# aik2mlj/polyffusion

Hardware: AMD Instinct MI355X
Metric: denoising steps/sec (8-bar prmat2c, batch 16) (higher is better)
Workload: dtype bf16x3; 1 GPU; sdf_chd8bar cond generation, batch 16 per GPU, 1000-step DDPM sampler loop body (BASELINE.json configs[1]); weights: deterministic synthetic, 41.08M params; global_batch=16, parallelism=batch-shard x1

## Files before the change

### polyffusion_amd/csrc/conv_common.h

```cpp
#pragma once
#include <type_traits>

#include "pf_internal.h"

namespace pf {

typedef x3_t x3x8 __attribute__((ext_vector_type(8)));
typedef unsigned int u32x4 __attribute__((ext_vector_type(4)));

template <int OFF>
__device__ __forceinline__ x3x8 lds_read128(unsigned addr) {
  u32x4 v;
  constexpr int HI = OFF & ~0xFFFF, LO = OFF & 0xFFFF;
  if constexpr (HI != 0) addr += HI;
  asm volatile("ds_read_b128 %0, %1 offset:%2" : "=v"(v) : "v"(addr), "n"(LO));
  return __builtin_bit_cast(x3x8, v);
}
__device__ __forceinline__ __amdgpu_buffer_rsrc_t dma_resource(const void* base) {
  return __builtin_amdgcn_make_buffer_rsrc(const_cast<void*>(base), 0, 0x7fffffff, 0x00020000);
}
__device__ __forceinline__ void dma16(__amdgpu_buffer_rsrc_t rs, int voff, int soff, void* lds_wave_base) {
  __builtin_amdgcn_raw_ptr_buffer_load_lds(rs, (__attribute__((address_space(3))) void*)lds_wave_base, 16, voff, soff, 0, 0);
}

template <int N>
__device__ __forceinline__ void lgkm_wait() { asm volatile("s_waitcnt lgkmcnt(%0)" ::"n"(N)); }
template <int I, int N, class F>
__device__ __forceinline__ void static_for(F&& f) {
  if constexpr (I < N) { f(std::integral_constant<int, I>{}); static_for<I + 1, N>(f); }
}


struct FastDiv { unsigned mul, shr; };
static inline FastDiv make_fastdiv(int d) {
  if (d <= 1) return FastDiv{0u, 0u};
  unsigned l = 31u - (unsigned)__builtin_clz((unsigned)d);
  if (d & (d - 1)) ++l;
  const unsigned p = 31u + l;
  return FastDiv{(unsigned)(((1ull << p) + (unsigned)d - 1u) / (unsigned)d), p - 32u};
}
__device__ __forceinline__ int fdiv(int x, FastDiv f) { return f.mul ? (int)(__umulhi((unsigned)x, f.mul) >> f.shr) : x; }

struct ConvP {
  const float* x0; const float* x1; int c0, c1;
  int B, Hin, Win, Hout, Wout;
  const void* w; int N, Npad;
  const float* sc; const float* sh; const float* mean; const float* rstd;
  const float* bias; const float* sbias; int ld_sbias; const float* res; int ld_res;
  const long long* sb_rows; int sb_nrows;
  int geglu;
  float* out; int ld_out;
  float* stats;
  int tiles_x, tiles_y, nt;
  FastDiv d_tx, d_ty, d_nt, d_ks;
  int fold, fold_py, fold_px;
  const float* sx0; const float* sx1; int sc0, sc1;
  const void* sw; const float* bias2;
  void* out_planes;
  void* qkv;
  int pp;
  int ksplit; float* partial;
  const float* gn_s0; const float* gn_s1; int gn_t0, gn_t1;
  const float* gn_gamma; const float* gn_beta; float gn_eps; int gn_groups;
  int x1_bmod;
  unsigned* amax;
  int pad_br;
};

__device__ __forceinline__ void conv_shared_x1(ConvP& p, int b) {
  if (p.x1_bmod > 0) {
    const size_t d = (size_t)(b - b % p.x1_bmod);
    if (p.x1) p.x1 -= d * ((size_t)p.Hin * p.Win * p.c1);
    if (p.sx1) p.sx1 -= d * ((size_t)p.Hout * p.Wout * p.sc1);
    if (p.gn_s1) p.gn_s1 -= d * ((size_t)p.gn_t1 * p.c1 * 2);
  }
}

static inline void conv_fill_divs(ConvP& p) {
  p.d_tx = make_fastdiv(p.tiles_x); p.d_ty = make_fastdiv(p.tiles_y); p.d_nt = make_fastdiv(p.nt); p.d_ks = make_fastdiv(p.ksplit);
}

template <int NTHREADS>
__device__ __forceinline__ void gn_fused_prologue(const ConvP& p, int b, int tid_wg, int hw, double* scratch) {
  const int cin = p.c0 + p.c1, gs = cin / p.gn_groups;
  for (int c = tid_wg; c < cin; c += NTHREADS) {
    const float* s; int T, C, cl;
    if (c < p.c0) { s = p.gn_s0; T = p.gn_t0; C = p.c0; cl = c; } else { s = p.gn_s1; T = p.gn_t1; C = p.c1; cl = c - p.c0; }
    double a = 0.0, q = 0.0;
    for (int t0 = 0; t0 < T; t0 += 8) {
      float2 vv[8];
#pragma unroll
      for (int j = 0; j < 8; ++j)
        vv[j] = *reinterpret_cast<const float2*>(s + (((size_t)b * T + min(t0 + j, T - 1)) * C + cl) * 2);
#pragma unroll
      for (int j = 0; j < 8; ++j)
        if (t0 + j < T) { a += vv[j].x; q += vv[j].y; }
    }
    scratch[2 * c] = a; scratch[2 * c + 1] = q;
  }
  __syncthreads();
  float* scw = const_cast<float*>(p.sc) + (size_t)b * cin;
  float* shw = const_cast<float*>(p.sh) + (size_t)b * cin;
  for (int c = tid_wg; c < cin; c += NTHREADS) {
    const int g0 = (c / gs) * gs;
    double a = 0.0, q = 0.0;
    for (int j = 0; j < gs; ++j) { a += scratch[2 * (g0 + j)]; q += scratch[2 * (g0 + j) + 1]; }
    const double cnt = (double)gs * hw;
    const double mean = a / cnt;
    double var = q / cnt - mean * mean;
    if (var < 0.0) var = 0.0;
    const double rstd = 1.0 / sqrt(var + (double)p.gn_eps);
    const double ga = p.gn_gamma[c];
    scw[c] = (float)(rstd * ga);
    shw[c] = (float)((double)p.gn_beta[c] - mean * rstd * ga);
  }
  __threadfence_block();
  __syncthreads();
}

__device__ __forceinline__ void amax_acc(unsigned& m, float v) { m = max(m, __float_as_uint(v) & 0x7fffffffu); }
__device__ __forceinline__ void amax_acc4(unsigned& m, f32x4 v) { amax_acc(m, v[0]); amax_acc(m, v[1]); amax_acc(m, v[2]); amax_acc(m, v[3]); }
__device__ __forceinline__ void amax_flush(unsigned* slot, unsigned m) {
  if (!slot) return;
#pragma unroll
  for (int o = 32; o >= 1; o >>= 1) m = max(m, (unsigned)__shfl_xor((int)m, o));
  if ((threadIdx.x & 63) == 0 && m) atomicMax(slot, m);
}

__device__ __forceinline__ float silu_f(float v) { return v * __builtin_amdgcn_rcpf(1.0f + __expf(-v)); }
__device__ __forceinline__ float erf_as_f(float x) {
  const float ax = fabsf(x);
  const float t = __builtin_amdgcn_rcpf(fmaf(0.3275911f, ax, 1.0f));
  float pq = fmaf(1.061405429f, t, -1.453152027f);
  pq = fmaf(pq, t, 1.421413741f);
  pq = fmaf(pq, t, -0.284496736f);
  pq = fmaf(pq, t, 0.254829592f);
  const float y = 1.0f - pq * t * __expf(-ax * ax);
  return copysignf(y, x);
}
__device__ __forceinline__ float gelu_erf_f(float g) { return 0.5f * g * (1.0f + erf_as_f(g * 0.70710678118654752440f)); }

__device__ __forceinline__ void store_out(const ConvP& p, size_t idx, float v) { p.out[idx] = v; }
__device__ __forceinline__ const float* sbias_row(const ConvP& p, int b) {
  if (!p.sbias) return nullptr;
  long long r = b;
  if (p.sb_rows) { r = p.sb_rows[b]; r = r < 0 ? 0 : (r >= p.sb_nrows ? p.sb_nrows - 1 : r); }
  return p.sbias + (size_t)r * p.ld_sbias;
}
__device__ __forceinline__ size_t out_pixel(const ConvP& p, int b, int oy, int ox) {
  if (p.fold) return ((size_t)b * (2 * p.Hout) + 2 * oy + p.fold_py) * (size_t)(2 * p.Wout) + 2 * ox + p.fold_px;
  return ((size_t)b * p.Hout + oy) * p.Wout + ox;
}

__device__ __forceinline__ void quad_transpose_s1(f32x4& a, int lane) {
  const bool p1 = lane & 1;
  float s0 = p1 ? a[0] : a[1], s1 = p1 ? a[2] : a[3];
  float r0 = __builtin_bit_cast(float, __builtin_amdgcn_mov_dpp(__builtin_bit_cast(int, s0), 0xB1, 0xF, 0xF, true));
  float r1 = __builtin_bit_cast(float, __builtin_amdgcn_mov_dpp(__builtin_bit_cast(int, s1), 0xB1, 0xF, 0xF, true));
  if (p1) { a[0] = r0; a[2] = r1; } else { a[1] = r0; a[3] = r1; }
}
__device__ __forceinline__ void quad_transpose_s2(f32x4& a, int lane) {
  const bool p2 = lane & 2;
  float s0 = p2 ? a[0] : a[2], s1 = p2 ? a[1] : a[3];
  float r0 = __builtin_bit_cast(float, __builtin_amdgcn_mov_dpp(__builtin_bit_cast(int, s0), 0x4E, 0xF, 0xF, true));
  float r1 = __builtin_bit_cast(float, __builtin_amdgcn_mov_dpp(__builtin_bit_cast(int, s1), 0x4E, 0xF, 0xF, true));
  if (p2) { a[0] = r0; a[1] = r1; } else { a[2] = r0; a[3] = r1; }
}
__device__ __forceinline__ void quad_transpose(f32x4& a, int lane) { quad_transpose_s1(a, lane); quad_transpose_s2(a, lane); }
__device__ __forceinline__ float quad_sum(float v) {
  v += __builtin_bit_cast(float, __builtin_amdgcn_mov_dpp(__builtin_bit_cast(int, v), 0xB1, 0xF, 0xF, true));
  v += __builtin_bit_cast(float, __builtin_amdgcn_mov_dpp(__builtin_bit_cast(int, v), 0x4E, 0xF, 0xF, true));
  return v;
}

template <int TH, int TW, int BN, int FM, int FN, int NWM = 2>
__device__ __forceinline__ void conv_epilogue(const ConvP& p, f32x16 (&acc)[FM][FN], int b, int oy0, int ox0, int n0,
                                              int wm, int wn, int lane, int tid, float* red, bool active = true) {
  constexpr int WM = TH * TW / NWM, WN = BN / 2;
  unsigned am = 0;
  if (!active) {
    if (p.stats && !p.partial) { __syncthreads(); __syncthreads(); }
    return;
  }
  if (p.partial) {
#pragma unroll
    for (int fm = 0; fm < FM; ++fm)
#pragma unroll
      for (int r = 0; r < 16; ++r) {
        const int row = (r & 3) + 8 * (r >> 2) + 4 * (lane >> 5);
        const int pp = wm * WM + fm * 32 + row;
        const int oy = oy0 + pp / TW, ox = ox0 + pp % TW;
        if (oy >= p.Hout || ox >= p.Wout) continue;
        const size_t m = out_pixel(p, b, oy, ox);
#pragma unroll
        for (int fn = 0; fn < FN; ++fn) {
          const int n = n0 + wn * WN + fn * 32 + (lane & 31);
          if (n < p.N) p.partial[m * p.N + n] = acc[fm][fn][r];
        }
      }
    return;
  }
  x3_t* pq = static_cast<x3_t*>(p.out_planes);
  size_t pq_plane = (size_t)p.B * p.Hout * p.Wout * p.ld_out;
  int pq_ld = p.ld_out, pq_n0 = p.geglu ? n0 / 2 : n0, pq_n = p.geglu ? p.N / 2 : p.N;
  if (p.qkv) {
    const int C = p.N / 3, which = n0 / C;
    pq = nullptr;
    if (C % BN == 0 && which < 2) {
      pq_plane = (size_t)p.B * p.Wout * C;
      pq = static_cast<x3_t*>(p.qkv) + (size_t)(2 * which) * pq_plane;
      pq_ld = C; pq_n0 = n0 - which * C; pq_n = C;
    }
  }
  if constexpr (TH == 1) if (pq) {
    const float* sb = p.qkv ? nullptr : sbias_row(p, b);
    const float* resp = p.qkv ? nullptr : p.res;
    typedef x3_t x3x8_t __attribute__((ext_vector_type(8)));
    const int L = p.Wout;
    const int bno = p.geglu ? BN / 2 : BN;
    const int pitch = bno + 8;
    __syncthreads();
#pragma unroll
    for (int fm = 0; fm < FM; ++fm) {
      if (p.geglu) {
        if constexpr (FN == 2) {
          const int nv = n0 + wn * WN + (lane & 31);
          const float bv = p.bias ? p.bias[nv] : 0.f, bg = p.bias ? p.bias[nv + 32] : 0.f;
#pragma unroll
          for (int r = 0; r < 16; ++r) {
            const int rl = wm * WM + fm * 32 + (r & 3) + 8 * (r >> 2) + 4 * (lane >> 5);
            red[rl * pitch + wn * (WN / 2) + (lane & 31)] = (acc[fm][0][r] + bv) * gelu_erf_f(acc[fm][1][r] + bg);
          }
        }
      } else {
#pragma unroll
        for (int fn = 0; fn < FN; ++fn) {
          const int cl = wn * WN + fn * 32 + (lane & 31);
#pragma unroll
          for (int r = 0; r < 16; ++r) {
            const int rl = wm * WM + fm * 32 + (r & 3) + 8 * (r >> 2) + 4 * (lane >> 5);
            red[rl * pitch + cl] = acc[fm][fn][r];
          }
        }
      }
    }
    __syncthreads();
    constexpr int NT = NWM * 128, ITER = TH * TW * (BN / 8) / NT;
    const int cpr = bno / 8;
    const int col = (tid % cpr) * 8, row0 = tid / cpr, rstep = NT / cpr;
    const bool cok = pq_n0 + col < pq_n;
    const int n = n0 + col;
    f32x4 ba = {0.f, 0.f, 0.f, 0.f}, bc = ba;
    if (!p.geglu && cok) {
      if (p.bias) { ba += *reinterpret_cast<const f32x4*>(p.bias + n); bc += *reinterpret_cast<const f32x4*>(p.bias + n + 4); }
      if (sb) { ba += *reinterpret_cast<const f32x4*>(sb + n); bc += *reinterpret_cast<const f32x4*>(sb + n + 4); }
    }
    f32x4 ra[ITER], rc[ITER];
#pragma unroll
    for (int it = 0; it < ITER; ++it) {
      const int rl = row0 + it * rstep;
      ra[it] = ba; rc[it] = bc;
      if (resp && cok && rl < TH * TW && ox0 + rl < L) {
        const float* rp = resp + ((size_t)b * L + ox0 + rl) * p.ld_res + n;
        ra[it] += *reinterpret_cast<const f32x4*>(rp); rc[it] += *reinterpret_cast<const f32x4*>(rp + 4);
      }
    }
#pragma unroll
    for (int it = 0; it < ITER; ++it) {
      const int rl = row0 + it * rstep;
      if (!cok || rl >= TH * TW || ox0 + rl >= L) continue;
      const f32x4 a = *reinterpret_cast<const f32x4*>(red + rl * pitch + col) + ra[it];
      const f32x4 c = *reinterpret_cast<const f32x4*>(red + rl * pitch + col + 4) + rc[it];
      if (p.amax) { amax_acc4(am, a); amax_acc4(am, c); }
      typedef x3_t x3x4_t __attribute__((ext_vector_type(4)));
      const x3x4_t ha = __builtin_convertvector(a, x3x4_t), hc = __builtin_convertvector(c, x3x4_t);
      const x3x4_t la = __builtin_convertvector(a - __builtin_convertvector(ha, f32x4), x3x4_t);
      const x3x4_t lc = __builtin_convertvector(c - __builtin_convertvector(hc, f32x4), x3x4_t);
      const x3x8_t hi = __builtin_shufflevector(ha, hc, 0, 1, 2, 3, 4, 5, 6, 7);
      const x3x8_t lo = __builtin_shufflevector(la, lc, 0, 1, 2, 3, 4, 5, 6, 7);
      const size_t o = ((size_t)b * L + ox0 + rl) * pq_ld + pq_n0 + col;
// ... 252 lines not shown
```

### polyffusion_amd/csrc/conv_wino.hip

```cpp
#include "conv_common.h"

namespace pf {

typedef x3_t x3x4 __attribute__((ext_vector_type(4)));

#ifdef PF_TRACE
__device__ unsigned long long g_wtrace[3 * 256];
#define WTR() do { if (trace_on && tslot < 255) { g_wtrace[tbase + tslot++] = __builtin_amdgcn_s_memtime(); } } while (0)
#define WTR_DECL() const bool trace_on = (threadIdx.x == 0) && (blockIdx.x == 0 || blockIdx.x == gridDim.x / 2 || blockIdx.x == gridDim.x - 1); \
                   const int tbase = blockIdx.x == 0 ? 0 : (blockIdx.x == gridDim.x - 1 ? 512 : 256); int tslot = 0; (void)tbase
#else
#define WTR() do {} while (0)
#define WTR_DECL() do {} while (0)
#endif

constexpr int WPP = 36, WRP = 18 * WPP + 8, WHALO = 18 * WRP;
constexpr int WINO_LDS = 4 * 2 * 4 * 16 * 64 * 4;

__device__ __forceinline__ void lds_barrier() {
  asm volatile("s_waitcnt lgkmcnt(0)" ::: "memory");
  __builtin_amdgcn_s_barrier();
  asm volatile("" ::: "memory");
}

template <class T>
__device__ __forceinline__ const T* uniform_ptr(const T* q) {
  const unsigned long long v = reinterpret_cast<unsigned long long>(q);
  const unsigned lo = __builtin_amdgcn_readfirstlane((unsigned)v), hi = __builtin_amdgcn_readfirstlane((unsigned)(v >> 32));
  return reinterpret_cast<const T*>(((unsigned long long)hi << 32) | lo);
}

__device__ __forceinline__ __amdgpu_buffer_rsrc_t rsrc_or_empty(const void* q) {
  return __builtin_amdgcn_make_buffer_rsrc(const_cast<void*>(q), 0, q ? 0x7fffffff : 0, 0x00020000);
}
__device__ __forceinline__ const float* sbias_row_scalar(const ConvP& p, int b) {
  if (!p.sbias) return nullptr;
  long long r = b;
  if (p.sb_rows) {
    typedef const long long __attribute__((address_space(4))) * cptr;
    r = *((cptr)(unsigned long long)(p.sb_rows + b));
    r = r < 0 ? 0 : (r >= p.sb_nrows ? p.sb_nrows - 1 : r);
  }
  return p.sbias + (size_t)r * p.ld_sbias;
}

__device__ __forceinline__ void wino_epilogue(const ConvP& p, f32x16 (&acc)[4][2][2], unsigned char* smem_all, int b, int oy0, int ox0, int n0,
                                              int ty_t, int tx_t, int wave, int lane, int tid, const float* sb, bool trace_on = false, int tbase = 0, int tslot = 0) {
  (void)trace_on; (void)tbase; (void)tslot;
  const int fh = wave >> 1, fnb = wave & 1;
  const int c8 = lane & 7, tl = lane >> 3;
  const int n = n0 + fnb * 32 + c8 * 4;
  const int pix0 = (b * p.Hout + oy0 + 8 * fh) * p.Wout + ox0 + 2 * tl;
  auto pix = [&](int u, int pp, int q) { return pix0 + (2 * u + pp) * p.Wout + q; };
  const __amdgpu_buffer_rsrc_t rsRes = rsrc_or_empty(uniform_ptr(p.res)), rsOut = rsrc_or_empty(uniform_ptr(p.out));
  f32x4 rr[4][2][2];
#pragma unroll
  for (int u = 0; u < 4; ++u)
#pragma unroll
    for (int pp = 0; pp < 2; ++pp)
#pragma unroll
      for (int q = 0; q < 2; ++q)
        rr[u][pp][q] = __builtin_bit_cast(f32x4, __builtin_amdgcn_raw_buffer_load_b128(rsRes, (pix(u, pp, q) * p.ld_res + n) * 4, 0, 0));
  const f32x4 cba = __builtin_bit_cast(f32x4, __builtin_amdgcn_raw_buffer_load_b128(rsrc_or_empty(uniform_ptr(p.bias)), n * 4, 0, 0));
  const f32x4 cbb = __builtin_bit_cast(f32x4, __builtin_amdgcn_raw_buffer_load_b128(rsrc_or_empty(uniform_ptr(sb)), n * 4, 0, 0));
  const f32x4 cbc = __builtin_bit_cast(f32x4, __builtin_amdgcn_raw_buffer_load_b128(rsrc_or_empty(uniform_ptr(p.bias2)), n * 4, 0, 0));
  lds_barrier();
  float* X = reinterpret_cast<float*>(smem_all);
#pragma unroll
  for (int h = 0; h < 2; ++h)
#pragma unroll
    for (int nb = 0; nb < 2; ++nb) {
      const int blk = h * 2 + nb;
#pragma unroll
      for (int r = 0; r < 16; ++r) {
        const float s0 = acc[0][h][nb][r] + acc[1][h][nb][r] + acc[2][h][nb][r];
        const float s1 = acc[1][h][nb][r] - acc[2][h][nb][r] - acc[3][h][nb][r];
        X[((((wave * 2 + 0) * 4 + blk) * 16 + r) * 64) + lane] = s0;
        X[((((wave * 2 + 1) * 4 + blk) * 16 + r) * 64) + lane] = s1;
      }
      __builtin_amdgcn_sched_barrier(0);
    }
  WTR();
  lds_barrier();
  WTR();
  const f32x4 cb4 = cba + cbb + cbc;
  f32x4 s1 = {0.f, 0.f, 0.f, 0.f}, s2 = s1;
  unsigned am = 0;
  const float* Xr = X + (tl & 3) * 64 + ((tl >> 2) & 1) * 32 + c8 * 4;
#pragma unroll
  for (int u = 0; u < 4; ++u)
#pragma unroll
    for (int q = 0; q < 2; ++q) {
      f32x4 sv[4];
#pragma unroll
      for (int i = 0; i < 4; ++i) sv[i] = *reinterpret_cast<const f32x4*>(Xr + ((((i * 2 + q) * 4 + wave) * 16 + 4 * u) * 64));
#pragma unroll
      for (int pp = 0; pp < 2; ++pp) {
        f32x4 v = pp == 0 ? sv[0] + sv[1] + sv[2] : sv[1] - sv[2] - sv[3];
        v = PF_X3_UNSCALE(v) + cb4 + rr[u][pp][q];
        __builtin_amdgcn_raw_buffer_store_b128(__builtin_bit_cast(u32x4, v), rsOut, (pix(u, pp, q) * p.ld_out + n) * 4, 0, 0);
        if (p.amax) amax_acc4(am, v);
        s1 += v; s2 += v * v;
      }
    }
  WTR();
  amax_flush(p.amax, am);
  if (p.stats) {
    lds_barrier();
    float* red = reinterpret_cast<float*>(smem_all);
    *reinterpret_cast<f32x4*>(red + (wave * 64 + lane) * 8) = s1;
    *reinterpret_cast<f32x4*>(red + (wave * 64 + lane) * 8 + 4) = s2;
    lds_barrier();
    if (tid < 64) {
      const int nb = tid >> 5, cc = (tid & 31) >> 2, e = tid & 3;
      float a0 = 0.f, a1 = 0.f;
#pragma unroll
      for (int h = 0; h < 2; ++h)
#pragma unroll
        for (int t8 = 0; t8 < 8; ++t8) {
          const float* q = red + ((h * 2 + nb) * 64 + t8 * 8 + cc) * 8 + e;
          a0 += q[0]; a1 += q[4];
        }
      const int tile = ty_t * p.tiles_x + tx_t;
      float* dst = p.stats + (((size_t)b * (p.tiles_x * p.tiles_y) + tile) * p.N + n0 + tid) * 2;
      dst[0] = a0; dst[1] = a1;
    }
  }
  WTR();
}

typedef float f32x2_ __attribute__((ext_vector_type(2)));
__device__ __forceinline__ f32x2_ silu2(f32x2_ v) {
  f32x2_ t = v * -1.44269504088896340736f;
  t[0] = __builtin_amdgcn_exp2f(t[0]); t[1] = __builtin_amdgcn_exp2f(t[1]);
  t = t + 1.0f;
  t[0] = __builtin_amdgcn_rcpf(t[0]); t[1] = __builtin_amdgcn_rcpf(t[1]);
  return v * t;
}

__device__ __forceinline__ f32x2_ pk_sub(f32x2_ a, f32x2_ b) { f32x2_ d; asm("v_pk_add_f32 %0, %1, %2 neg_lo:[0,1] neg_hi:[0,1]" : "=v"(d) : "v"(a), "v"(b)); return d; }
__device__ __forceinline__ f32x2_ pk_fma(f32x2_ a, f32x2_ b, f32x2_ c) { f32x2_ d; asm("v_pk_fma_f32 %0, %1, %2, %3" : "=v"(d) : "v"(a), "v"(b), "v"(c)); return d; }
__device__ __forceinline__ f32x4 sub4(f32x4 a, f32x4 b) {
  const f32x2_ l = pk_sub(f32x2_{a[0], a[1]}, f32x2_{b[0], b[1]}), h = pk_sub(f32x2_{a[2], a[3]}, f32x2_{b[2], b[3]});
  return f32x4{l[0], l[1], h[0], h[1]};
}
__device__ __forceinline__ f32x4 fma4(f32x4 a, f32x2_ s2, f32x4 c) {
  const f32x2_ l = pk_fma(f32x2_{a[0], a[1]}, s2, f32x2_{c[0], c[1]}), h = pk_fma(f32x2_{a[2], a[3]}, s2, f32x2_{c[2], c[3]});
  return f32x4{l[0], l[1], h[0], h[1]};
}

typedef x3_t x3x2 __attribute__((ext_vector_type(2)));
typedef float f32x2 __attribute__((ext_vector_type(2)));
struct SplitK { unsigned c0, c1; };
__device__ __forceinline__ SplitK split_consts() {
#ifdef PF_X3_F16
  SplitK k{0x0000BC00u, 0xBC000000u};
#else
  SplitK k{0x0000BF80u, 0xBF800000u};
#endif
  asm volatile("" : "+s"(k.c0), "+s"(k.c1));
  return k;
}
__device__ __forceinline__ float x3_sub_hi(x3x2 hp, unsigned c, float v) {
#ifdef PF_X3_F16
  return __builtin_amdgcn_fdot2(hp, __builtin_bit_cast(x3x2, c), v, false);
#else
  return __builtin_amdgcn_fdot2_f32_bf16(hp, __builtin_bit_cast(x3x2, c), v, false);
#endif
}
__device__ __forceinline__ void split4(f32x4 v, x3x4& hi, x3x4& lo, SplitK k) {
  const x3x2 h01 = __builtin_convertvector(f32x2{v[0], v[1]}, x3x2), h23 = __builtin_convertvector(f32x2{v[2], v[3]}, x3x2);
  const float l0 = x3_sub_hi(h01, k.c0, v[0]), l1 = x3_sub_hi(h01, k.c1, v[1]), l2 = x3_sub_hi(h23, k.c0, v[2]), l3 = x3_sub_hi(h23, k.c1, v[3]);
  const x3x2 q01 = __builtin_convertvector(f32x2{l0, l1}, x3x2), q23 = __builtin_convertvector(f32x2{l2, l3}, x3x2);
  hi = __builtin_shufflevector(h01, h23, 0, 1, 2, 3);
  lo = __builtin_shufflevector(q01, q23, 0, 1, 2, 3);
}

template <int DUMMY>
__global__ __launch_bounds__(256, 1) void conv_wino_pipe_kernel(ConvP p) {
  extern __shared__ __attribute__((aligned(16))) unsigned char smem_all[];
  WTR_DECL();
  WTR();
  constexpr int WIMG = WHALO + 1024;
  float* H0 = reinterpret_cast<float*>(smem_all) + 1024;
  const int tid = threadIdx.x, lane = tid & 63;
  const int wave = __builtin_amdgcn_readfirstlane(tid >> 6);

  int lid;
  {
    const int nwg = gridDim.x, orig = blockIdx.x;
    const int xcd = orig & 7, q = nwg >> 3, r = nwg & 7;
    lid = __builtin_amdgcn_readfirstlane((xcd < r ? xcd * (q + 1) : r * (q + 1) + (xcd - r) * q) + (orig >> 3));
  }
  int mt = __builtin_amdgcn_readfirstlane(fdiv(lid, p.d_nt));
  const int nti = lid - mt * p.nt;
  int t = __builtin_amdgcn_readfirstlane(fdiv(mt, p.d_tx));
  const int tx_t = mt - t * p.tiles_x; mt = t;
  const int b = __builtin_amdgcn_readfirstlane(fdiv(mt, p.d_ty));
  const int ty_t = mt - b * p.tiles_y;
  const int n0 = nti * 64, oy0 = ty_t * 16, ox0 = tx_t * 16;
  conv_shared_x1(p, b);
  const int cin = p.c0 + p.c1, nchunk = cin / 32, KK = cin / 16;
  const float* sbp = sbias_row_scalar(p, b);

  if (p.gn_s0) gn_fused_prologue<256>(p, b, tid, p.Hin * p.Win, reinterpret_cast<double*>(smem_all));

  const int sub = tid & 7;
  int* gpL = reinterpret_cast<int*>(H0 + WIMG + WHALO) + tid;
  int gpr[11];
  const int bpix = b * p.Hin * p.Win;
#pragma unroll
  for (int it = 0; it < 11; ++it) {
    const int pix = min((tid >> 3) + 32 * it, 323);
    const int row = (int)__umul24(pix, 57) >> 10, col = pix - (int)__umul24(row, 18);
    const int iy = oy0 - 1 + row, ix = ox0 - 1 + col;
    const bool inside = (unsigned)iy < (unsigned)p.Hin && (unsigned)ix < (unsigned)p.Win;
    const int gpix = inside ? (int)__umul24(iy, p.Win) + ix + 1 : 0;
    const int real4 = (int)__umul24(row, WRP / 4) + (int)__umul24(col, WPP / 4) + (sub ^ ((row >> 1) & 1));
    const int lo4 = inside ? 256 + real4 : tid;
    if (!inside) {
      *reinterpret_cast<f32x4*>(H0 + real4 * 4) = f32x4{0.f, 0.f, 0.f, 0.f};
      *reinterpret_cast<f32x4*>(H0 + WIMG + real4 * 4) = f32x4{0.f, 0.f, 0.f, 0.f};
    }
    gpr[it] = gpix | (lo4 << 20);
    gpL[it * 256] = gpr[it];
  }
  const __amdgpu_buffer_rsrc_t rsSc = dma_resource(uniform_ptr(p.sc + (size_t)b * cin)), rsSh = dma_resource(uniform_ptr(p.sh + (size_t)b * cin));
  float* scL = reinterpret_cast<float*>(gpL - tid + 11 * 256);
  float* shL = scL + cin;
  const float* px0 = uniform_ptr(p.x0);
  const float* px1 = uniform_ptr(p.x1);
  f32x4 ra[11], vsc, vsh;
  auto scRead = [&](int ct) {
    vsc = *reinterpret_cast<const f32x4*>(scL + ct * 32 + sub * 4);
    vsh = *reinterpret_cast<const f32x4*>(shL + ct * 32 + sub * 4);
  };
  int gq = 0, gst = 0;
  auto gpRead = [&](int pi) { gq = gpL[pi * 256]; };
  auto haloFetch = [&](int ct, int gpv, int skip = 0) -> f32x4 {
    const int cg = ct * 32;
    const bool first = cg < p.c0;
    const __amdgpu_buffer_rsrc_t rs = dma_resource(first ? px0 : px1);
    const int cs4 = (first ? p.c0 : p.c1) * 4, co4 = (first ? cg : cg - p.c0) * 4 + bpix * cs4;
    const int gpix = (gpv & 0xFFFFF) - 1;
    const int vo = ((int)__umul24(gpix, cs4) + sub * 16) | (gpix & (int)0x80000000u) | skip;
    return __builtin_bit_cast(f32x4, __builtin_amdgcn_raw_buffer_load_b128(rs, vo, co4, 0));
  };
  auto haloLoad = [&](int pi, int ct, int gpv, int skip = 0) { ra[pi] = haloFetch(ct, gpv, skip); };
  auto stageWhole = [&](f32x4 r, f32x4 sc4, f32x4 sh4, int gpv, float* Ht) {
    r = r * sc4 + sh4;
    const f32x2_ a = silu2(f32x2_{r[0], r[1]}), c2 = silu2(f32x2_{r[2], r[3]});
    *reinterpret_cast<f32x4*>(Ht - 1024 + (((unsigned)gpv >> 20) << 2)) = f32x4{a[0], a[1], c2[0], c2[1]};
  };
  auto scLoad = [&](int ct) {
    vsc = __builtin_bit_cast(f32x4, __builtin_amdgcn_raw_buffer_load_b128(rsSc, sub * 16, ct * 128, 0));
    vsh = __builtin_bit_cast(f32x4, __builtin_amdgcn_raw_buffer_load_b128(rsSh, sub * 16, ct * 128, 0));
  };
  auto stageA = [&](int pi) {
    gst = gpL[pi * 256];
    const f32x2_ a = silu2(f32x2_{ra[pi][0], ra[pi][1]} * f32x2_{vsc[0], vsc[1]} + f32x2_{vsh[0], vsh[1]});
    ra[pi][0] = a[0]; ra[pi][1] = a[1];
  };
  auto stageB = [&](int pi, float* Ht) {
    const f32x2_ a = silu2(f32x2_{ra[pi][2], ra[pi][3]} * f32x2_{vsc[2], vsc[3]} + f32x2_{vsh[2], vsh[3]});
    ra[pi][2] = a[0]; ra[pi][3] = a[1];
    *reinterpret_cast<f32x4*>(Ht - 1024 + (((unsigned)gst >> 20) << 2)) = ra[pi];
  };

  const int m = lane & 31, g = lane >> 5, tyl = m >> 3, txl = m & 7;
  const int ax = wave == 0 ? 0 : (wave == 2 ? 2 : 1);
  const int ay = wave == 0 ? 2 : (wave == 1 ? 2 : (wave == 2 ? 1 : 3));
  const float sigma = wave == 1 ? 1.f : -1.f;
  int ox_, oy_;
  {
    const int rx = 2 * tyl + ax, ry = 2 * tyl + ay;
    ox_ = rx * WRP + (2 * txl) * WPP + (((2 * g) ^ ((rx >> 1) & 1)) << 2);
    oy_ = ry * WRP + (2 * txl) * WPP + (((2 * g) ^ ((ry >> 1) & 1)) << 2);
    asm volatile("" : "+v"(ox_), "+v"(oy_));
  }
  const SplitK spk = split_consts();
  f32x2_ sig2 = {sigma, sigma};
  asm volatile("" : "+v"(sig2));
  f32x4 rwx[2], rwy[2], tt[4];
  x3x4 fh_[2][4][2], fl_[2][4][2];
  auto fragRead = [&](const float* Hn, int s, int h, int e, int b2) {
    int ex = ox_, ey = oy_;
    if (e) { asm volatile("v_xor_b32 %0, 4, %1" : "=v"(ex) : "v"(ox_)); asm volatile("v_xor_b32 %0, 4, %1" : "=v"(ey) : "v"(oy_)); }
#pragma unroll
    for (int bb = 0; bb < 2; ++bb) {
      rwx[bb] = *reinterpret_cast<const f32x4*>(Hn + ex + ((2 * b2 + bb) * WPP + s * 16 + h * 8 * WRP));
      rwy[bb] = *reinterpret_cast<const f32x4*>(Hn + ey + ((2 * b2 + bb) * WPP + s * 16 + h * 8 * WRP));
    }
  };
  auto fragT = [&](int b2) {
#pragma unroll
    for (int bb = 0; bb < 2; ++bb) tt[2 * b2 + bb] = fma4(rwy[bb], sig2, rwx[bb]);
  };
  auto fragV = [&](int set, int j, int e) {
    const f32x4 v = j == 0 ? sub4(tt[0], tt[2]) : (j == 1 ? tt[1] + tt[2] : (j == 2 ? sub4(tt[2], tt[1]) : sub4(tt[1], tt[3])));
    split4(v, fh_[set][j][e], fl_[set][j][e], spk);
  };

  const __amdgpu_buffer_rsrc_t rsW = dma_resource(uniform_ptr(static_cast<const x3_t*>(p.w) + ((size_t)wave * KK * p.nt + nti) * 8192));
  const int wstep = p.nt * 16384;
  x3x8 bh[4][2], bl[4][2];
  auto wLoad = [&](int j, int kk) {
#pragma unroll
    for (int nb = 0; nb < 2; ++nb) {
      bh[j][nb] = __builtin_bit_cast(x3x8, __builtin_amdgcn_raw_buffer_load_b128(rsW, lane * 16, kk * wstep + ((j * 2 + nb) * 2 + 0) * 1024, 0));
      bl[j][nb] = __builtin_bit_cast(x3x8, __builtin_amdgcn_raw_buffer_load_b128(rsW, lane * 16, kk * wstep + ((j * 2 + nb) * 2 + 1) * 1024, 0));
    }
  };

  auto wLoad1 = [&](int j, int nb, bool lo, int kk, int skip) {
    if (lo) bl[j][nb] = __builtin_bit_cast(x3x8, __builtin_amdgcn_raw_buffer_load_b128(rsW, (lane * 16) | skip, kk * wstep + ((j * 2 + nb) * 2 + 1) * 1024, 0));
    else bh[j][nb] = __builtin_bit_cast(x3x8, __builtin_amdgcn_raw_buffer_load_b128(rsW, (lane * 16) | skip, kk * wstep + ((j * 2 + nb) * 2 + 0) * 1024, 0));
  };
  f32x16 acc[4][2][2];

#define SB() __builtin_amdgcn_sched_barrier(0)
  {
    const int c1 = min(1, nchunk - 1);
#pragma unroll
    for (int pi = 0; pi < 11; ++pi) haloLoad(pi, 0, gpr[pi]);
    scLoad(0);
    const f32x4 vsc0 = vsc, vsh0 = vsh;
    f32x4 rb[3];
#pragma unroll
    for (int pi = 0; pi < 3; ++pi) rb[pi] = haloFetch(c1, gpr[pi]);
    scLoad(c1);
#pragma unroll
    for (int j = 0; j < 4; ++j) wLoad(j, 0);
    float tsc[4], tsh[4];
#pragma unroll
    for (int i = 0; i < 4; ++i) {
      const int c = min(tid + 256 * i, cin - 1);
      tsc[i] = p.sc[(size_t)b * cin + c]; tsh[i] = p.sh[(size_t)b * cin + c];
    }
    WTR();
    SB();
    {
      x3x8 z8;
#pragma unroll
      for (int e = 0; e < 8; ++e) z8[e] = (x3_t)0.f;
      asm volatile("" : "+v"(z8));
      const f32x16 z16 = {0.f, 0.f, 0.f, 0.f, 0.f, 0.f, 0.f, 0.f, 0.f, 0.f, 0.f, 0.f, 0.f, 0.f, 0.f, 0.f};
#pragma unroll
      for (int j = 0; j < 4; ++j)
#pragma unroll
        for (int h = 0; h < 2; ++h)
#pragma unroll
          for (int nb = 0; nb < 2; ++nb) {
            asm volatile("" : "+v"(z8));
            acc[j][h][nb] = x3_mfma_32x32x16(z8, z8, z16, 0, 0, 0);
          }
    }
#pragma unroll
    for (int i = 0; i < 4; ++i)
      if (tid + 256 * i < cin) { scL[tid + 256 * i] = tsc[i]; shL[tid + 256 * i] = tsh[i]; }
    SB();
#pragma unroll
    for (int pi = 0; pi < 11; ++pi) stageWhole(ra[pi], vsc0, vsh0, gpr[pi], H0);
    WTR();
#pragma unroll
    for (int pi = 0; pi < 3; ++pi) stageWhole(rb[pi], vsc, vsh, gpr[pi], H0 + WIMG);
#pragma unroll
    for (int pi = 3; pi < 9; ++pi) haloLoad(pi, c1, gpr[pi]);
    WTR();
    __syncthreads();
    WTR();
#pragma unroll
    for (int e = 0; e < 2; ++e) {
      fragRead(H0, 0, 0, e, 0); fragT(0); fragRead(H0, 0, 0, e, 1); fragT(1);
#pragma unroll
      for (int j = 0; j < 4; ++j) fragV(0, j, e);
    }
  }

  for (int chunk = 0; chunk < nchunk; ++chunk) {
    const int c1 = min(chunk + 1, nchunk - 1), c2 = min(chunk + 2, nchunk - 1);
    const int skip1 = chunk + 1 < nchunk ? 0 : (int)0x80000000u, skip2 = chunk + 2 < nchunk ? 0 : (int)0x80000000u;
    float* Hcur = H0 + (chunk & 1) * WIMG;
    float* Hnxt = H0 + ((chunk + 1) & 1) * WIMG;
    static_for<0, 4>([&](auto qc) {
      constexpr int QS = decltype(qc)::value, s = QS >> 1, h = QS & 1;
      constexpr int QN = (QS + 1) & 3, sn = QN >> 1, hn = QN & 1;
      const float* Hn = QS == 3 ? Hnxt : Hcur;
      float* Ht = QS == 3 ? Hcur : Hnxt;
      constexpr int sp0 = QS == 3 ? 0 : 3 * QS + 3, spn = QS == 2 ? 2 : 3;
      constexpr int lp0 = QS == 0 ? 9 : 3 * (QS - 1), lpn = QS == 0 ? 2 : 3;
      const int lct = QS == 0 ? c1 : c2;
      WTR();
      if constexpr (QS == 3) {
        asm volatile("s_waitcnt lgkmcnt(0)" ::: "memory");
        __builtin_amdgcn_s_barrier();
        asm volatile("" ::: "memory");
      }
      SB();
      static_for<0, 24>([&](auto kc) {
        constexpr int k = decltype(kc)::value, j = k / 6, kind = (k % 6) >> 1, nb = k & 1;
        const x3x8 ah = __builtin_shufflevector(fh_[h][j][0], fh_[h][j][1], 0, 1, 2, 3, 4, 5, 6, 7);
        const x3x8 al = __builtin_shufflevector(fl_[h][j][0], fl_[h][j][1], 0, 1, 2, 3, 4, 5, 6, 7);
        if constexpr (kind == 0) acc[j][h][nb] = x3_mfma_32x32x16(al, bh[j][nb], acc[j][h][nb], 0, 0, 0);
        else if constexpr (kind == 1) acc[j][h][nb] = x3_mfma_32x32x16(ah, bl[j][nb], acc[j][h][nb], 0, 0, 0);
        else acc[j][h][nb] = x3_mfma_32x32x16(ah, bh[j][nb], acc[j][h][nb], 0, 0, 0);
        SB();
        if constexpr (k == 0 || k == 8) fragRead(Hn, sn, hn, k / 8, 0);
        if constexpr (k == 2 || k == 10) { fragT(0); fragRead(Hn, sn, hn, k / 8, 1); }
        if constexpr (k == 4 || k == 12) { fragT(1); fragV(hn, 0, k / 8); }
        if constexpr (k == 5 || k == 6 || k == 7) fragV(hn, k - 4, 0);
        if constexpr (k == 13 || k == 14 || k == 15) fragV(hn, k - 12, 1);
        if constexpr (k >= 16 && k < 16 + 2 * spn) {
          constexpr int pi = sp0 + (k - 16) / 2;
          if constexpr (((k - 16) & 1) == 0) stageA(pi); else stageB(pi, Ht);
        }
        if constexpr (k == 3 || k == 9 || k == 11) {
          constexpr int li = k == 3 ? 0 : (k == 9 ? 1 : 2);
          if constexpr (li < lpn) haloLoad(lp0 + li, lct, gq, QS == 0 ? skip1 : skip2);
        }
        if constexpr (k == 1 || k == 7 || k == 9) {
          constexpr int li = k == 1 ? 0 : (k == 7 ? 1 : 2);
          if constexpr (li < lpn) gpRead(lp0 + li);
        }
        if constexpr (k == 15) scRead(QS == 3 ? c2 : c1);
        if constexpr (h == 1 && (k % 6) >= 2) wLoad1(j, k & 1, (k % 6) < 4, s == 0 ? chunk * 2 + 1 : c1 * 2, s == 0 ? 0 : skip1);
        SB();
      });
    });
  }
#undef SB
  WTR();
#ifdef PF_TRACE
  wino_epilogue(p, acc, smem_all, b, oy0, ox0, n0, ty_t, tx_t, wave, lane, tid, sbp, trace_on, tbase, tslot);
#else
  wino_epilogue(p, acc, smem_all, b, oy0, ox0, n0, ty_t, tx_t, wave, lane, tid, sbp);
#endif
}

bool conv_wino_eligible(const pf_conv_args& a) {
  return a.wino > 0 && a.w_wino && a.precision == PF_PREC_BF16X3 && a.ks == 3 && a.stride == 1 && !a.ups && !a.ups_fold && a.prologue == 1 &&
         a.hin % 16 == 0 && a.win % 16 == 0 && a.n % 64 == 0 && a.c0 % 32 == 0 && a.c1 % 32 == 0 && !a.geglu && !a.out_planes && !a.qkv_planes &&
         a.c0 + a.c1 <= 1024 && a.hin * a.win < (1 << 20) &&
         (long long)a.batch * a.hin * a.win * (a.c0 > a.c1 ? a.c0 : a.c1) * 4 < (1ll << 31) &&
         (long long)a.batch * a.hin * a.win * (a.ld_out > a.ld_res ? a.ld_out : a.ld_res) * 4 < (1ll << 31) &&
         !a.skip_w && (a.ld_out & 3) == 0 && (!a.res || (a.ld_res & 3) == 0);
}

int launch_conv_wino(const pf_conv_args& a, hipStream_t stream) {
  ConvP p;
  memset(&p, 0, sizeof p);
  p.x0 = a.x0; p.x1 = a.x1; p.c0 = a.c0; p.c1 = a.c1;
  p.B = a.batch; p.Hin = a.hin; p.Win = a.win; p.Hout = a.hin; p.Wout = a.win;
  p.w = a.w_wino; p.N = a.n; p.Npad = a.n;
  p.sc = a.sc; p.sh = a.sh;
  p.bias = a.bias; p.sbias = a.sbias; p.ld_sbias = a.ld_sbias; p.res = a.res; p.ld_res = a.ld_res;
  p.sb_rows = reinterpret_cast<const long long*>(a.sbias_rows); p.sb_nrows = a.sbias_nrows;
  p.out = a.out; p.ld_out = a.ld_out; p.stats = a.stats_out;
  p.ksplit = 1;
  if (a.gn_stats0) {
    p.gn_s0 = a.gn_stats0; p.gn_t0 = a.gn_tiles0; p.gn_s1 = a.gn_stats1; p.gn_t1 = a.gn_tiles1;
    p.gn_gamma = a.gn_gamma; p.gn_beta = a.gn_beta; p.gn_eps = a.gn_eps; p.gn_groups = a.gn_groups;
  }
  p.x1_bmod = a.x1_bmod;
  p.amax = static_cast<unsigned*>(a.absmax_slot);
  p.tiles_x = a.win / 16; p.tiles_y = a.hin / 16; p.nt = a.n / 64;
  conv_fill_divs(p);
  const int grid = p.B * p.tiles_y * p.tiles_x * p.nt;
  auto kern = conv_wino_pipe_kernel<0>;
  static std::atomic<uint64_t> attr_done{0};
  if (int rc = set_max_lds_once(reinterpret_cast<const void*>(kern), WINO_LDS, attr_done)) return rc;
  hipLaunchKernelGGL(kern, dim3(grid), dim3(256), WINO_LDS, stream, p);
  PF_CHECK_HIP(hipGetLastError());
  return PF_OK;
}

#ifdef PF_TRACE
extern "C" int pf_debug_wino_trace_read(unsigned long long* dst, int n) {
  return hipMemcpyFromSymbol(dst, HIP_SYMBOL(g_wtrace), (size_t)n * 8) == hipSuccess ? 0 : -1;
}
extern "C" int pf_debug_wino_trace_clear() {
  static unsigned long long z[3 * 256];
  return hipMemcpyToSymbol(HIP_SYMBOL(g_wtrace), z, sizeof z) == hipSuccess ? 0 : -1;
}
#endif

static inline unsigned short wf2bf_rne(float f) {
  unsigned int u; memcpy(&u, &f, 4);
  u += 0x7FFFu + ((u >> 16) & 1u);
  return (unsigned short)(u >> 16);
}
static inline float wbf2f(unsigned short h) { unsigned int u = (unsigned int)h << 16; float f; memcpy(&f, &u, 4); return f; }

bool pack_wino_bf3(void* dst_, const float* src, int N, int K) {
  unsigned short* dst = (unsigned short*)dst_;
  bool fits = true;
  const int KK = K / 16, NT = N / 64;
  static const double G[4][3] = {{1.0, 0.0, 0.0}, {0.5, 0.5, 0.5}, {0.5, -0.5, 0.5}, {0.0, 0.0, 1.0}};
  for (int n = 0; n < N; ++n)
    for (int k = 0; k < K; ++k) {
      const float* g = src + ((size_t)n * K + k) * 9;
      double Gg[4][3];
      for (int i = 0; i < 4; ++i)
        for (int c = 0; c < 3; ++c) Gg[i][c] = G[i][0] * g[0 * 3 + c] + G[i][1] * g[1 * 3 + c] + G[i][2] * g[2 * 3 + c];
      for (int i = 0; i < 4; ++i)
        for (int j = 0; j < 4; ++j) {
          const double ud = Gg[i][0] * G[j][0] + Gg[i][1] * G[j][1] + Gg[i][2] * G[j][2];
          const float v = (float)ud;
#ifdef PF_X3_F16
          const float vs = fminf(fmaxf(v * PF_X3_WS, -65504.f), 65504.f);
          fits = fits && vs == v * PF_X3_WS;
          const _Float16 fh = (_Float16)vs, fl = (_Float16)(vs - (float)fh);
          unsigned short hi, lo;
          memcpy(&hi, &fh, 2); memcpy(&lo, &fl, 2);
#else
          const unsigned short hi = wf2bf_rne(v);
          const unsigned short lo = wf2bf_rne(v - wbf2f(hi));
#endif
          const int kk = k / 16, ln = ((k % 16) / 8) * 32 + (n % 32), e = k % 8, ntile = n / 64, nb = (n % 64) / 32;
          const size_t frag = ((((size_t)i * KK + kk) * NT + ntile) * 4 + j) * 2 + nb;
          dst[((frag * 2 + 0) * 64 + ln) * 8 + e] = hi;
          dst[((frag * 2 + 1) * 64 + ln) * 8 + e] = lo;
        }
    }
  return fits;
}

}
```

Baseline: 212.8 steps/s.

## Hoist weight/halo prologue loads, split SiLU staging, use cross-lane stats reduction

Moves the first weight fragment loads ahead of the GroupNorm prologue and issues the halo, scale and shift loads before the LDS index-table setup, so global-memory latency overlaps setup work. Splits the SiLU activation staging into four finer steps (exp2, then rcp) spread across more MFMA slots. Replaces the epilogue's LDS-based GroupNorm stats reduction with DPP and permlane swaps plus a small extra LDS exchange between wave halves, which removes one barrier and the serial 64-thread summation. It costs more live registers in the prologue and adds a small LDS region.

```diff
diff --git a/polyffusion_amd/csrc/conv_common.h b/polyffusion_amd/csrc/conv_common.h
--- a/polyffusion_amd/csrc/conv_common.h
+++ b/polyffusion_amd/csrc/conv_common.h
@@ -120,12 +120,13 @@
 
 __device__ __forceinline__ void amax_acc(unsigned& m, float v) { m = max(m, __float_as_uint(v) & 0x7fffffffu); }
 __device__ __forceinline__ void amax_acc4(unsigned& m, f32x4 v) { amax_acc(m, v[0]); amax_acc(m, v[1]); amax_acc(m, v[2]); amax_acc(m, v[3]); }
-__device__ __forceinline__ void amax_flush(unsigned* slot, unsigned m) {
+__device__ __forceinline__ void amax_flush(unsigned* slot, unsigned m, int lane) {
   if (!slot) return;
 #pragma unroll
   for (int o = 32; o >= 1; o >>= 1) m = max(m, (unsigned)__shfl_xor((int)m, o));
-  if ((threadIdx.x & 63) == 0 && m) atomicMax(slot, m);
-}
+  if (lane == 0 && m) atomicMax(slot, m);
+}
+__device__ __forceinline__ void amax_flush(unsigned* slot, unsigned m) { amax_flush(slot, m, threadIdx.x & 63); }
 
 __device__ __forceinline__ float silu_f(float v) { return v * __builtin_amdgcn_rcpf(1.0f + __expf(-v)); }
 __device__ __forceinline__ float erf_as_f(float x) {
diff --git a/polyffusion_amd/csrc/conv_wino.hip b/polyffusion_amd/csrc/conv_wino.hip
--- a/polyffusion_amd/csrc/conv_wino.hip
+++ b/polyffusion_amd/csrc/conv_wino.hip
@@ -15,7 +15,8 @@
 #endif
 
 constexpr int WPP = 36, WRP = 18 * WPP + 8, WHALO = 18 * WRP;
-constexpr int WINO_LDS = 4 * 2 * 4 * 16 * 64 * 4;
+constexpr int WINO_XCH = 4 * 2 * 4 * 16 * 64 * 4;
+constexpr int WINO_LDS = WINO_XCH + 64 * 2 * 4;
 
 __device__ __forceinline__ void lds_barrier() {
   asm volatile("s_waitcnt lgkmcnt(0)" ::: "memory");
@@ -45,8 +46,10 @@
 }
 
 __device__ __forceinline__ void wino_epilogue(const ConvP& p, f32x16 (&acc)[4][2][2], unsigned char* smem_all, int b, int oy0, int ox0, int n0,
-                                              int ty_t, int tx_t, int wave, int lane, int tid, const float* sb, bool trace_on = false, int tbase = 0, int tslot = 0) {
+                                              int ty_t, int tx_t, int wave, const float* sb, bool trace_on = false, int tbase = 0, int tslot = 0) {
   (void)trace_on; (void)tbase; (void)tslot;
+  int lane;
+  asm volatile("v_mbcnt_lo_u32_b32 %0, -1, 0\n\tv_mbcnt_hi_u32_b32 %0, -1, %0" : "=v"(lane));
   const int fh = wave >> 1, fnb = wave & 1;
   const int c8 = lane & 7, tl = lane >> 3;
   const int n = n0 + fnb * 32 + c8 * 4;
@@ -104,26 +107,33 @@
       }
     }
   WTR();
-  amax_flush(p.amax, am);
+  amax_flush(p.amax, am, lane);
   if (p.stats) {
+    auto row8 = [](float v) {
+      return v + __builtin_bit_cast(float, __builtin_amdgcn_update_dpp(0, __builtin_bit_cast(int, v), 0x128 , 0xf, 0xf, false));
+    };
+    auto pair16 = [](float x, float y) {
+      const auto r = __builtin_amdgcn_permlane16_swap(__builtin_bit_cast(unsigned, x), __builtin_bit_cast(unsigned, y), false, false);
+      const unsigned r0 = r[0], r1 = r[1];
+      return __builtin_bit_cast(float, r0) + __builtin_bit_cast(float, r1);
+    };
+    auto pair32 = [](float x, float y) {
+      const auto r = __builtin_amdgcn_permlane32_swap(__builtin_bit_cast(unsigned, x), __builtin_bit_cast(unsigned, y), false, false);
+      const unsigned r0 = r[0], r1 = r[1];
+      return __builtin_bit_cast(float, r0) + __builtin_bit_cast(float, r1);
+    };
+    const float c1 = pair32(pair16(row8(s1[0]), row8(s1[1])), pair16(row8(s1[2]), row8(s1[3])));
+    const float c2 = pair32(pair16(row8(s2[0]), row8(s2[1])), pair16(row8(s2[2]), row8(s2[3])));
+    const int ch = fnb * 32 + c8 * 4 + (lane >> 4);
+    const bool owner = (lane & 8) == 0;
+    float2* red = reinterpret_cast<float2*>(smem_all + WINO_XCH) + ch;
+    if (fh == 1 && owner) *red = float2{c1, c2};
     lds_barrier();
-    float* red = reinterpret_cast<float*>(smem_all);
-    *reinterpret_cast<f32x4*>(red + (wave * 64 + lane) * 8) = s1;
-    *reinterpret_cast<f32x4*>(red + (wave * 64 + lane) * 8 + 4) = s2;
-    lds_barrier();
-    if (tid < 64) {
-      const int nb = tid >> 5, cc = (tid & 31) >> 2, e = tid & 3;
-      float a0 = 0.f, a1 = 0.f;
-#pragma unroll
-      for (int h = 0; h < 2; ++h)
-#pragma unroll
-        for (int t8 = 0; t8 < 8; ++t8) {
-          const float* q = red + ((h * 2 + nb) * 64 + t8 * 8 + cc) * 8 + e;
-          a0 += q[0]; a1 += q[4];
-        }
+    if (fh == 0 && owner) {
+      const float2 o = *red;
       const int tile = ty_t * p.tiles_x + tx_t;
-      float* dst = p.stats + (((size_t)b * (p.tiles_x * p.tiles_y) + tile) * p.N + n0 + tid) * 2;
-      dst[0] = a0; dst[1] = a1;
+      float2* dst = reinterpret_cast<float2*>(p.stats + (((size_t)b * (p.tiles_x * p.tiles_y) + tile) * p.N + n0 + ch) * 2);
+      *dst = float2{c1 + o.x, c2 + o.y};
     }
   }
   WTR();
@@ -203,28 +213,29 @@
   const int cin = p.c0 + p.c1, nchunk = cin / 32, KK = cin / 16;
   const float* sbp = sbias_row_scalar(p, b);
 
+  const __amdgpu_buffer_rsrc_t rsW = dma_resource(uniform_ptr(static_cast<const x3_t*>(p.w) + ((size_t)wave * KK * p.nt + nti) * 8192));
+  const int wstep = p.nt * 16384;
+  x3x8 bh[4][2], bl[4][2];
+  auto wLoad = [&](int j, int kk) {
+#pragma unroll
+    for (int nb = 0; nb < 2; ++nb) {
+      bh[j][nb] = __builtin_bit_cast(x3x8, __builtin_amdgcn_raw_buffer_load_b128(rsW, lane * 16, kk * wstep + ((j * 2 + nb) * 2 + 0) * 1024, 0));
+      bl[j][nb] = __builtin_bit_cast(x3x8, __builtin_amdgcn_raw_buffer_load_b128(rsW, lane * 16, kk * wstep + ((j * 2 + nb) * 2 + 1) * 1024, 0));
+    }
+  };
+
+  auto wLoad1 = [&](int j, int nb, bool lo, int kk, int skip) {
+    if (lo) bl[j][nb] = __builtin_bit_cast(x3x8, __builtin_amdgcn_raw_buffer_load_b128(rsW, (lane * 16) | skip, kk * wstep + ((j * 2 + nb) * 2 + 1) * 1024, 0));
+    else bh[j][nb] = __builtin_bit_cast(x3x8, __builtin_amdgcn_raw_buffer_load_b128(rsW, (lane * 16) | skip, kk * wstep + ((j * 2 + nb) * 2 + 0) * 1024, 0));
+  };
+#pragma unroll
+  for (int j = 0; j < 4; ++j) wLoad(j, 0);
+
   if (p.gn_s0) gn_fused_prologue<256>(p, b, tid, p.Hin * p.Win, reinterpret_cast<double*>(smem_all));
 
   const int sub = tid & 7;
   int* gpL = reinterpret_cast<int*>(H0 + WIMG + WHALO) + tid;
-  int gpr[11];
   const int bpix = b * p.Hin * p.Win;
-#pragma unroll
-  for (int it = 0; it < 11; ++it) {
-    const int pix = min((tid >> 3) + 32 * it, 323);
-    const int row = (int)__umul24(pix, 57) >> 10, col = pix - (int)__umul24(row, 18);
-    const int iy = oy0 - 1 + row, ix = ox0 - 1 + col;
-    const bool inside = (unsigned)iy < (unsigned)p.Hin && (unsigned)ix < (unsigned)p.Win;
-    const int gpix = inside ? (int)__umul24(iy, p.Win) + ix + 1 : 0;
-    const int real4 = (int)__umul24(row, WRP / 4) + (int)__umul24(col, WPP / 4) + (sub ^ ((row >> 1) & 1));
-    const int lo4 = inside ? 256 + real4 : tid;
-    if (!inside) {
-      *reinterpret_cast<f32x4*>(H0 + real4 * 4) = f32x4{0.f, 0.f, 0.f, 0.f};
-      *reinterpret_cast<f32x4*>(H0 + WIMG + real4 * 4) = f32x4{0.f, 0.f, 0.f, 0.f};
-    }
-    gpr[it] = gpix | (lo4 << 20);
-    gpL[it * 256] = gpr[it];
-  }
   const __amdgpu_buffer_rsrc_t rsSc = dma_resource(uniform_ptr(p.sc + (size_t)b * cin)), rsSh = dma_resource(uniform_ptr(p.sh + (size_t)b * cin));
   float* scL = reinterpret_cast<float*>(gpL - tid + 11 * 256);
   float* shL = scL + cin;
@@ -256,16 +267,67 @@
     vsc = __builtin_bit_cast(f32x4, __builtin_amdgcn_raw_buffer_load_b128(rsSc, sub * 16, ct * 128, 0));
     vsh = __builtin_bit_cast(f32x4, __builtin_amdgcn_raw_buffer_load_b128(rsSh, sub * 16, ct * 128, 0));
   };
-  auto stageA = [&](int pi) {
-    gst = gpL[pi * 256];
-    const f32x2_ a = silu2(f32x2_{ra[pi][0], ra[pi][1]} * f32x2_{vsc[0], vsc[1]} + f32x2_{vsh[0], vsh[1]});
-    ra[pi][0] = a[0]; ra[pi][1] = a[1];
-  };
-  auto stageB = [&](int pi, float* Ht) {
-    const f32x2_ a = silu2(f32x2_{ra[pi][2], ra[pi][3]} * f32x2_{vsc[2], vsc[3]} + f32x2_{vsh[2], vsh[3]});
-    ra[pi][2] = a[0]; ra[pi][3] = a[1];
-    *reinterpret_cast<f32x4*>(Ht - 1024 + (((unsigned)gst >> 20) << 2)) = ra[pi];
-  };
+  f32x2_ sq = {0.f, 0.f};
+  auto stageQ = [&](int pi, int q, float* Ht) {
+    const int e0 = (q >> 1) * 2;
+    if ((q & 1) == 0) {
+      if (q == 0) gst = gpL[pi * 256];
+      const f32x2_ v = f32x2_{ra[pi][e0], ra[pi][e0 + 1]} * f32x2_{vsc[e0], vsc[e0 + 1]} + f32x2_{vsh[e0], vsh[e0 + 1]};
+      ra[pi][e0] = v[0]; ra[pi][e0 + 1] = v[1];
+      const f32x2_ t = v * -1.44269504088896340736f;
+      sq[0] = __builtin_amdgcn_exp2f(t[0]); sq[1] = __builtin_amdgcn_exp2f(t[1]);
+    } else {
+      f32x2_ t = sq + 1.0f;
+      t[0] = __builtin_amdgcn_rcpf(t[0]); t[1] = __builtin_amdgcn_rcpf(t[1]);
+      const f32x2_ a = f32x2_{ra[pi][e0], ra[pi][e0 + 1]} * t;
+      ra[pi][e0] = a[0]; ra[pi][e0 + 1] = a[1];
+      if (q == 3) *reinterpret_cast<f32x4*>(Ht - 1024 + (((unsigned)gst >> 20) << 2)) = ra[pi];
+    }
+  };
+
+  const int pc1 = min(1, nchunk - 1);
+  scLoad(0);
+  const f32x4 vsc0 = vsc, vsh0 = vsh;
+  scLoad(pc1);
+  float tsc[4], tsh[4];
+#pragma unroll
+  for (int i = 0; i < 4; ++i) {
+    tsc[i] = tsh[i] = 0.f;
+    if (i == 0 || cin > 256 * i) {
+      const int c = tid + 256 * i, vo = (c * 4) | (c < cin ? 0 : (int)0x80000000u);
+      tsc[i] = __builtin_bit_cast(float, __builtin_amdgcn_raw_buffer_load_b32(rsSc, vo, 0, 0));
+      tsh[i] = __builtin_bit_cast(float, __builtin_amdgcn_raw_buffer_load_b32(rsSh, vo, 0, 0));
+    }
+  }
+  int prow[11], pcol[11], gpx[11];
+  f32x4 rb[3];
+#pragma unroll
+  for (int it = 0; it < 11; ++it) {
+    const int pix = min((tid >> 3) + 32 * it, 323);
+    const int row = (int)__umul24(pix, 57) >> 10, col = pix - (int)__umul24(row, 18);
+    const int iy = oy0 - 1 + row, ix = ox0 - 1 + col;
+    const bool inside = (unsigned)iy < (unsigned)p.Hin && (unsigned)ix < (unsigned)p.Win;
+    gpx[it] = inside ? (int)__umul24(iy, p.Win) + ix + 1 : 0;
+    prow[it] = row; pcol[it] = col;
+    haloLoad(it, 0, gpx[it]);
+  }
+#pragma unroll
+  for (int pi = 0; pi < 3; ++pi) rb[pi] = haloFetch(pc1, gpx[pi]);
+  __builtin_amdgcn_sched_barrier(0);
+  int gpr[11];
+#pragma unroll
+  for (int it = 0; it < 11; ++it) {
+    const int row = prow[it], col = pcol[it];
+    const bool inside = gpx[it] != 0;
+    const int real4 = (int)__umul24(row, WRP / 4) + (int)__umul24(col, WPP / 4) + (sub ^ ((row >> 1) & 1));
+    const int lo4 = inside ? 256 + real4 : tid;
+    if (!inside) {
+      *reinterpret_cast<f32x4*>(H0 + real4 * 4) = f32x4{0.f, 0.f, 0.f, 0.f};
+      *reinterpret_cast<f32x4*>(H0 + WIMG + real4 * 4) = f32x4{0.f, 0.f, 0.f, 0.f};
+    }
+    gpr[it] = gpx[it] | (lo4 << 20);
+    gpL[it * 256] = gpr[it];
+  }
 
   const int m = lane & 31, g = lane >> 5, tyl = m >> 3, txl = m & 7;
   const int ax = wave == 0 ? 0 : (wave == 2 ? 2 : 1);
@@ -301,42 +363,11 @@
     split4(v, fh_[set][j][e], fl_[set][j][e], spk);
   };
 
-  const __amdgpu_buffer_rsrc_t rsW = dma_resource(uniform_ptr(static_cast<const x3_t*>(p.w) + ((size_t)wave * KK * p.nt + nti) * 8192));
-  const int wstep = p.nt * 16384;
-  x3x8 bh[4][2], bl[4][2];
-  auto wLoad = [&](int j, int kk) {
-#pragma unroll
-    for (int nb = 0; nb < 2; ++nb) {
-      bh[j][nb] = __builtin_bit_cast(x3x8, __builtin_amdgcn_raw_buffer_load_b128(rsW, lane * 16, kk * wstep + ((j * 2 + nb) * 2 + 0) * 1024, 0));
-      bl[j][nb] = __builtin_bit_cast(x3x8, __builtin_amdgcn_raw_buffer_load_b128(rsW, lane * 16, kk * wstep + ((j * 2 + nb) * 2 + 1) * 1024, 0));
-    }
-  };
-
-  auto wLoad1 = [&](int j, int nb, bool lo, int kk, int skip) {
-    if (lo) bl[j][nb] = __builtin_bit_cast(x3x8, __builtin_amdgcn_raw_buffer_load_b128(rsW, (lane * 16) | skip, kk * wstep + ((j * 2 + nb) * 2 + 1) * 1024, 0));
-    else bh[j][nb] = __builtin_bit_cast(x3x8, __builtin_amdgcn_raw_buffer_load_b128(rsW, (lane * 16) | skip, kk * wstep + ((j * 2 + nb) * 2 + 0) * 1024, 0));
-  };
   f32x16 acc[4][2][2];
 
 #define SB() __builtin_amdgcn_sched_barrier(0)
   {
-    const int c1 = min(1, nchunk - 1);
-#pragma unroll
-    for (int pi = 0; pi < 11; ++pi) haloLoad(pi, 0, gpr[pi]);
-    scLoad(0);
-    const f32x4 vsc0 = vsc, vsh0 = vsh;
-    f32x4 rb[3];
-#pragma unroll
-    for (int pi = 0; pi < 3; ++pi) rb[pi] = haloFetch(c1, gpr[pi]);
-    scLoad(c1);
-#pragma unroll
-    for (int j = 0; j < 4; ++j) wLoad(j, 0);
-    float tsc[4], tsh[4];
-#pragma unroll
-    for (int i = 0; i < 4; ++i) {
-      const int c = min(tid + 256 * i, cin - 1);
-      tsc[i] = p.sc[(size_t)b * cin + c]; tsh[i] = p.sh[(size_t)b * cin + c];
-    }
+    const int c1 = pc1;
     WTR();
     SB();
     {
@@ -410,9 +441,9 @@
         if constexpr (k == 4 || k == 12) { fragT(1); fragV(hn, 0, k / 8); }
         if constexpr (k == 5 || k == 6 || k == 7) fragV(hn, k - 4, 0);
         if constexpr (k == 13 || k == 14 || k == 15) fragV(hn, k - 12, 1);
-        if constexpr (k >= 16 && k < 16 + 2 * spn) {
-          constexpr int pi = sp0 + (k - 16) / 2;
-          if constexpr (((k - 16) & 1) == 0) stageA(pi); else stageB(pi, Ht);
+        if constexpr (k >= 16) {
+          constexpr int nq = 4 * spn, q0 = (k - 16) * nq / 8, q1 = (k - 15) * nq / 8;
+          static_for<q0, q1>([&](auto qq) { constexpr int q = decltype(qq)::value; stageQ(sp0 + q / 4, q % 4, Ht); });
         }
         if constexpr (k == 3 || k == 9 || k == 11) {
           constexpr int li = k == 3 ? 0 : (k == 9 ? 1 : 2);
@@ -431,9 +462,9 @@
 #undef SB
   WTR();
 #ifdef PF_TRACE
-  wino_epilogue(p, acc, smem_all, b, oy0, ox0, n0, ty_t, tx_t, wave, lane, tid, sbp, trace_on, tbase, tslot);
+  wino_epilogue(p, acc, smem_all, b, oy0, ox0, n0, ty_t, tx_t, wave, sbp, trace_on, tbase, tslot);
 #else
-  wino_epilogue(p, acc, smem_all, b, oy0, ox0, n0, ty_t, tx_t, wave, lane, tid, sbp);
+  wino_epilogue(p, acc, smem_all, b, oy0, ox0, n0, ty_t, tx_t, wave, sbp);
 #endif
 }
 
```

Result: no change. 213.6 steps/s, median of 6 (+0.3%).
